# anyboby/Constrained-Model-Based-Policy-Optimization

Hardware: NVIDIA B200
Metric: model-rollout transitions/sec (higher is better)
Workload: dtype f16 (tcgen05 kind::f16, f32 accumulate)

## Files before the change

### constrained-model-based-policy-optimization_b200/csrc/common.cuh

```cuda
#pragma once
#include <cuda_runtime.h>
#include <stdint.h>
#include <stdio.h>
#include <string>
#include <vector>

#include "../../include/cmbpo_b200.h"

#define CMBPO_MAX_LAYERS 8
#define CMBPO_MAX_E 8
#define CMBPO_MAX_OBS 64
#define CMBPO_MAX_ACT 32

void cmbpo_set_error(const char* fmt, ...);

#define CUDA_TRY(expr)                                                                   \
    do {                                                                                 \
        cudaError_t _e = (expr);                                                         \
        if (_e != cudaSuccess) {                                                         \
            cmbpo_set_error("%s failed: %s (%s:%d)", #expr, cudaGetErrorString(_e), __FILE__, \
                            __LINE__);                                                   \
            return 1;                                                                    \
        }                                                                                \
    } while (0)
// ... 66 lines not shown
    ProfScope(cmbpo_ctx* c, int s) : ctx(c), slot(s), on(c->profile && s >= 0) {
        if (!on) return;
        ProfSlot& p = ctx->prof[slot];
        if (p.used == p.start.size()) {
            cudaEvent_t a, b;
            cudaEventCreate(&a); cudaEventCreate(&b);
            p.start.push_back(a); p.stop.push_back(b);
        }
        cudaEventRecord(p.start[p.used], ctx->stream);
    }
    ~ProfScope() {
        if (!on) return;
        ProfSlot& p = ctx->prof[slot];
        cudaEventRecord(p.stop[p.used], ctx->stream);
        p.used++;
    }
};

static inline int cdiv(int64_t a, int64_t b) { return (int)((a + b - 1) / b); }

int ens_forward_f32(cmbpo_ctx* ctx, const Net& net, const float* x, int64_t N, bool x_is_3d,
                    float* out_raw);
struct FusedStep;
int ens_forward_tc(cmbpo_ctx* ctx, Net& net, const float* x, int64_t N, float* out_raw,
                   int precision, const int64_t* n_dev = nullptr, const FusedStep* fz = nullptr);
bool ens_tc_fusable(const Net& net);
int ens_tc_fused_rp_shift(int obs_dim);
bool ens_tc_supported(const Net& net);
int ens_tc_prepare(cmbpo_ctx* ctx, Net& net);
int policy_pack_build(cmbpo_ctx* ctx);
void net_free(Net& n);
void train_free(cmbpo_ctx* ctx, int which);
int ens_forward(cmbpo_ctx* ctx, Net& net, const float* x, int64_t N, bool x_is_3d, float* out_raw,
                int precision, const int64_t* n_dev = nullptr);
```

### constrained-model-based-policy-optimization_b200/csrc/ens_tc.cu

```cuda
#include <cstring>
#include "tc_common.cuh"
#include "step_common.cuh"

using namespace tc;

namespace {

constexpr int NTHREADS = 640;
constexpr int TILE = 8192;
constexpr int STAGE = 4 * TILE;
constexpr int NSM = 5;
constexpr int W2SLOT = 16384;
constexpr int NS2 = 2;
constexpr int BIAS_SLOT = 4096;
constexpr int XA_BYTES = 16384;

struct Stage {
    int layer, n0, k0, rows, member;
    unsigned long long off;
};

struct TcParams {
    const uint8_t* wmain; unsigned long long main_bytes;
    const uint8_t* w2; unsigned long long w2_bytes;
    const float* bias; int bias_stride;
    int E, K0, KS0, Nout, NP, parts, cps;
    int fold;
    const float* x; long long N; int ldx;
    const long long* n_dev;
    const float *mu_in, *sig_in;
    float* out; long long out_member_stride;
    int ntiles;
    int member_act[CMBPO_MAX_E];
    FusedStep fz;
};

enum { W_FULL = 0, W_EMPTY = NSM, W2_FULL = 2 * NSM, W2_EMPTY = 2 * NSM + NS2, D_FULL = 2 * NSM + 2 * NS2,
       D_EMPTY = D_FULL + 2, H1_FULL = D_FULL + 4, H2_FULL = D_FULL + 5, H2_EMPTY = D_FULL + 7,
       OUT_FULL = D_FULL + 9, OUT_EMPTY = D_FULL + 10, X_FULL = D_FULL + 11, B_FULL = D_FULL + 12,
       B_EMPTY = D_FULL + 14, NBAR = D_FULL + 16 };
constexpr int HL_FULL = H2_FULL;
static_assert(H2_EMPTY == H2_FULL + 2, "HL_FULL spans the H2_FULL and H2_EMPTY pairs");
constexpr int SMEM_W2 = XA_BYTES + NSM * STAGE;
constexpr int SMEM_BIAS = SMEM_W2 + NS2 * W2SLOT;
constexpr int SMEM_IN_BYTES = 512;
constexpr int SMEM_BAR = SMEM_BIAS + 2 * BIAS_SLOT + SMEM_IN_BYTES;
constexpr int SMEM_TOTAL = SMEM_BAR + NBAR * 8 + 16;
constexpr int W2SLOT_F = 12288;
constexpr int FZ_STAGE = 12288, FZ_MISC = 5120;
constexpr int SMEM_BIAS_F = SMEM_W2 + NS2 * W2SLOT_F;
constexpr int SMEM_BAR_F = SMEM_BIAS_F + 2 * BIAS_SLOT + SMEM_IN_BYTES;
constexpr int SMEM_FZ = SMEM_BAR_F + NBAR * 8 + 16;
constexpr int SMEM_TOTAL_F = SMEM_FZ + FZ_STAGE + FZ_MISC;
static_assert(SMEM_FZ % 16 == 0 && SMEM_TOTAL_F + 1024 <= 232448, "fused shared-memory budget");

struct FzSmem {
    float *kl, *epv;
    int *member, *path;
    int* nonfin;
    float* spec;
    float *sig, *mu, *l2s;
    float* log_std;
    int* elite;
    unsigned char* state;
    int* flag;
};
__device__ __forceinline__ FzSmem fz_views(uint8_t* base) {
    FzSmem m;
    m.kl = reinterpret_cast<float*>(base);
    m.epv = nullptr;
// ... 96 lines not shown
            if (!c.deterministic)
                eps = f.state_eps ? f.state_eps[pth * O + dim] : philox_normal(f.seed, f.path_base + pth, t, RNG_STREAM_STATE, dim);
            RawTile raw(tbase, W, r0 + rr);
            const float ob = f.cur_obs[(base + rr) * O + dim];
            const float nx = env_dim_nx<true>(c, raw, dim, member, ob, eps);
            if (!f.rules.no_store) {
                f.rules.b.obs[row * O + dim] = ob;
                f.rules.b.nextobs[row * O + dim] = nx;
            }
            f.cur_obs[(base + rr) * O + dim] = nx;
        }
        if (!f.rules.no_store)
        for (int idx = etid; idx < RP * A; idx += 512) {
            const int rr = idx / A, i = idx - rr * A;
            if (sm.state[rr] != 1) continue;
            const long long pth = sm.path[rr], row = (long long)t * f.rules.B + pth;
            f.rules.b.act[row * A + i] = f.pi[(base + rr) * A + i];
            f.rules.b.mu[row * A + i] = f.mu[(base + rr) * A + i];
        }
        epi_bar();
    }
}


template <int FMT, int ACT>
__device__ __forceinline__ void drain32(uint32_t d_addr, const float* bias, uint32_t dst_addr,
                                        uint32_t d_empty, uint32_t dst_free, uint32_t dst_parity,
                                        bool rt_swish = false) {
    uint32_t r[32];
    tmem_ld32(d_addr, r);
    tmem_ld_wait();
    tc_fence_before();
    __syncwarp();
    if ((threadIdx.x & 31) == 0) mbar_arrive_a(d_empty);
    uint32_t q[16];
    float v[32];
    if (bias) {
#pragma unroll
        for (int i = 0; i < 32; i += 4) {
            const float4 b = *reinterpret_cast<const float4*>(bias + i);
            v[i] = __uint_as_float(r[i]) + b.x; v[i + 1] = __uint_as_float(r[i + 1]) + b.y;
            v[i + 2] = __uint_as_float(r[i + 2]) + b.z; v[i + 3] = __uint_as_float(r[i + 3]) + b.w;
        }
    } else {
#pragma unroll
        for (int i = 0; i < 32; ++i) v[i] = __uint_as_float(r[i]);
    }
#pragma unroll
    for (int i = 0; i < 32; ++i) {
        if (ACT == 0) {
            const float r = tanh_approx(v[i]);
            const float sw = fmaf(v[i], r, v[i]);
            v[i] = rt_swish ? sw : r;
        } else {
            v[i] = (ACT == CMBPO_ACT_SWISH) ? swish_half(v[i]) : tanh_approx(v[i]);
        }
    }
#pragma unroll
    for (int c = 0; c < 16; ++c) q[c] = Cvt<FMT>::pack(v[2 * c], v[2 * c + 1]);
    if (dst_free) { mbar_wait_a(dst_free, dst_parity); tc_fence_after(); }
    tmem_st16(dst_addr, q);
    tmem_st_wait();
    tc_fence_before();
}

template <int HD, int FMT, int ACT, int G, bool FUSE, int NMID = 0, int CL = 1, bool WO = false>
__global__ void __launch_bounds__(NTHREADS, 1) ens_mlp3_tc_kernel(const TcParams p) {
    static_assert(CL == 1 || (CL == 2 && G == 1 && !FUSE), "cluster pairs: ordinary ensembles only");
    static_assert(!FUSE || G == 1, "the fused step kernel exists for ordinary (ungrouped) ensembles");
    static_assert(NMID == 0 || (HD <= 256 && G == 1 && !FUSE), "deep variant: width <= 256, ungrouped");
    static_assert(!WO || (NMID > 0 && HD == 256 && CL == 1), "wide-output variant: deep nets at padded width 256");
    constexpr int W2S = FUSE ? W2SLOT_F : W2SLOT;
    constexpr int NC = HD / 64;
    constexpr int KP = HD / 64 / G;
    constexpr int CPM = NC / G;
    constexpr int TPS = KP < 4 ? KP : 4;
    constexpr int G0 = NC < 4 ? NC : 4;
    constexpr uint32_t COL_H1 = 0, COL_D = HD / 2, COL_H2 = COL_D + 128;
    constexpr uint32_t COL_HB = WO ? COL_H2 : COL_H2 + 64;
    constexpr int NHID = 1 + NMID;
    constexpr uint32_t COL_LAST = ((NMID + 1) & 1) ? COL_HB : COL_H1;
    extern __shared__ uint8_t smem_raw[];
    uint8_t* smem = reinterpret_cast<uint8_t*>((reinterpret_cast<uintptr_t>(smem_raw) + 1023) & ~uintptr_t(1023));
    uint8_t* sXA = smem;
    uint8_t* sW = smem + XA_BYTES;
    uint8_t* sW2 = smem + SMEM_W2;
    float* sBias = reinterpret_cast<float*>(smem + (FUSE ? SMEM_BIAS_F : SMEM_BIAS));
    float* sIn = sBias + 2 * BIAS_SLOT / 4;
    constexpr int BAR_OFF = FUSE ? SMEM_BAR_F : SMEM_BAR;
    uint64_t* bar = reinterpret_cast<uint64_t*>(smem + BAR_OFF);
// ... 226 lines not shown
                }
                ++m;
            }
        }
        }
        __syncwarp();
    }
    } else {
        asm volatile("setmaxnreg.inc.sync.aligned.u32 112;");
        const int wg = (warp - 4) >> 2;
        const uint32_t pair = (uint32_t)wg >> 1, half = (uint32_t)wg & 1;
        const int wq = hw_warp & 3;
        const int row = wq * 32 + lane;
        const uint32_t lane_base = (uint32_t)(wq * 32) << 16;
        const uint32_t bar_a = smem_u32(bar);
        uint32_t g = 0, m = 0, c1 = 0;
        int prev_e = 0; long long prev_grow = 0; uint32_t prev_m = 0; bool have_prev = false;
        int prev_tile = 0;
        const int etid = (int)threadIdx.x - 128;
        if (etid < 64) {
            sIn[etid] = (p.mu_in && etid < p.K0) ? p.mu_in[etid] : 0.f;
            sIn[64 + etid] = (p.mu_in && etid < p.K0) ? p.sig_in[etid] : 1.f;
        }
        epi_bar();
        FzSmem fsm;
        if (FUSE) {
            fsm = fz_views(smem + SMEM_FZ);
            const FusedStep& f = p.fz;
            for (int i = etid; i < f.c.D; i += 512) { fsm.sig[i] = f.c.sig_out[i]; fsm.mu[i] = f.c.mu_out[i]; fsm.l2s[i] = f.c.l2s_out[i]; }
            if (etid < f.A) fsm.log_std[etid] = f.log_std[etid];
            if (etid < f.n_elite && etid < 8) fsm.elite[etid] = f.c.elite[etid];
            epi_bar();
        }
        const int out_cw = (G > 1) ? p.NP : ((p.NP <= 64) ? 16 : 32);
        auto out_epilogue = [&]() {
            mbar_wait(bar + OUT_FULL, prev_m & 1);
            tc_fence_after();
            const int c_begin = wg * out_cw;
            uint32_t r[32];
            const bool mine = (G > 1) ? (wg < G && prev_e * G + wg < p.E) : (c_begin < p.NP);
            if (mine) {
                tmem_ld16(tmem + col_out + c_begin + lane_base, *reinterpret_cast<uint32_t(*)[16]>(&r[0]));
                if (out_cw == 32) tmem_ld16(tmem + col_out + c_begin + 16 + lane_base, *reinterpret_cast<uint32_t(*)[16]>(&r[16]));
                tmem_ld_wait();
            }
            tc_fence_before();
            __syncwarp();
            if (lane == 0) mbar_arrive(bar + OUT_EMPTY);
            if (FUSE) {
                const FusedStep& f = p.fz;
                if (mine) {
                    const float* b2 = p.bias + (long long)prev_e * p.bias_stride + (1 + NHID) * HD;
                    float* dst = f.raw_tiles + ((size_t)prev_tile * p.E + prev_e) * p.Nout * 128 + row;
#pragma unroll
                    for (int i = 0; i < 32; ++i) {
                        const int c = c_begin + i;
                        if (i < out_cw && c < p.Nout) __stcg(dst + (size_t)c * 128, __uint_as_float(r[i]) + __ldg(b2 + c));
                    }
                }
                __threadfence();
                epi_bar();
                if (etid == 0) {
                    const int old = atomicAdd(f.tile_cnt + prev_tile, 1);
                    const int last = (old == p.E - 1) ? 1 : 0;
                    if (last) f.tile_cnt[prev_tile] = 0;
                    *fsm.flag = last;
                }
                epi_bar();
                if (*fsm.flag) {
                    __threadfence();
                    fused_rows(f, fsm, prev_tile, n_rows, etid);
// ... 240 lines not shown
        for (int j = 0; j < NC; ++j)
            for (int kp = 0; kp < KPm; ++kp) {
                main_prog->push_back(Stage{lyr, (j % CPM) * 64, kp * 64, 64, j / CPM, off});
                off += TILE;
            }
    *main_bytes = off;
    off = 0;
    for (int j = 0; j < NC; ++j)
        for (int q = 0; q < parts; ++q) {
            w2_prog->push_back(Stage{nhid + 1, q * NPp, (j % CPM) * 64, NPp, j / CPM, off});
            off += (unsigned long long)NPp * 128;
        }
    *w2_bytes = off;
}

int chunks_per_w2_slot(int HD, int NP, int slot_bytes = W2SLOT) {
    int cps = slot_bytes / (NP * 128);
    int p2 = 1;
    while (p2 * 2 <= cps) p2 *= 2;
    const int NC = HD / 64;
    return p2 < NC ? p2 : NC;
}

template <int HD, int FMT, int ACT, int G = 1, bool FUSE = false, int NMID = 0, bool WO = false>
int launch_tc(cmbpo_ctx* ctx, const TcParams& p) {
    const int smem = (FUSE ? SMEM_TOTAL_F : SMEM_TOTAL) + 1024;
    static_assert(SMEM_TOTAL + 1024 <= 232448, "shared memory budget");
    auto kern = ens_mlp3_tc_kernel<HD, FMT, ACT, G, FUSE, NMID, 1, WO>;
    CUDA_TRY(cudaFuncSetAttribute(kern, cudaFuncAttributeMaxDynamicSharedMemorySize, smem));
    const long long units = (long long)p.ntiles * ((p.E + G - 1) / G);
    const int grid = units < ctx->sm_count ? (int)units : ctx->sm_count;
    kern<<<grid, NTHREADS, smem, ctx->stream>>>(p);
    ctx->launches++;
    CUDA_TRY(cudaGetLastError());
    return 0;
}

template <int HD, int FMT, int ACT>
int launch_tc_pairs(cmbpo_ctx* ctx, const TcParams& p) {
    const int smem = SMEM_TOTAL + 1024;
    auto kern = ens_mlp3_tc_kernel<HD, FMT, ACT, 1, false, 0, 2>;
    static int max_pairs = -1;
    cudaLaunchConfig_t cfg = {};
    cudaLaunchAttribute attr[1];
    attr[0].id = cudaLaunchAttributeClusterDimension;
    attr[0].val.clusterDim.x = 2; attr[0].val.clusterDim.y = 1; attr[0].val.clusterDim.z = 1;
    cfg.blockDim = dim3(NTHREADS); cfg.dynamicSmemBytes = smem; cfg.stream = ctx->stream;
    cfg.attrs = attr; cfg.numAttrs = 1;
    if (max_pairs < 0) {
        CUDA_TRY(cudaFuncSetAttribute(kern, cudaFuncAttributeMaxDynamicSharedMemorySize, smem));
        cfg.gridDim = dim3(2 * (ctx->sm_count / 2));
// ... 24 lines not shown

template <int HD, int FMT>
int launch_tc_act(cmbpo_ctx* ctx, const TcParams& p, int act) {
    if (act == 0) return launch_tc<HD, FMT, 0>(ctx, p);
    if (act == CMBPO_ACT_SWISH) return launch_tc<HD, FMT, CMBPO_ACT_SWISH>(ctx, p);
    return launch_tc<HD, FMT, CMBPO_ACT_TANH>(ctx, p);
}

template <int FMT, int ACT, int NMID>
int launch_tc_deep_out(cmbpo_ctx* ctx, const TcParams& p) {
    if (p.NP > 64) return launch_tc<256, FMT, ACT, 1, false, NMID, true>(ctx, p);
    return launch_tc<256, FMT, ACT, 1, false, NMID>(ctx, p);
}
template <int FMT>
int launch_tc_deep(cmbpo_ctx* ctx, const TcParams& p, int act, int nmid) {
    if (act == CMBPO_ACT_SWISH)
        return nmid == 1 ? launch_tc_deep_out<FMT, CMBPO_ACT_SWISH, 1>(ctx, p)
                         : launch_tc_deep_out<FMT, CMBPO_ACT_SWISH, 2>(ctx, p);
    return nmid == 1 ? launch_tc_deep_out<FMT, CMBPO_ACT_TANH, 1>(ctx, p)
                     : launch_tc_deep_out<FMT, CMBPO_ACT_TANH, 2>(ctx, p);
}

template <int FMT>
int launch_tc_grouped(cmbpo_ctx* ctx, const TcParams& p, int act) {
    if (act == 0) return launch_tc<512, FMT, 0, 4>(ctx, p);
    if (act == CMBPO_ACT_SWISH) return launch_tc<512, FMT, CMBPO_ACT_SWISH, 4>(ctx, p);
    return launch_tc<512, FMT, CMBPO_ACT_TANH, 4>(ctx, p);
}

template <int FMT>
int launch_tc_hd(cmbpo_ctx* ctx, const TcParams& p, int hd, int act) {
    if (hd == 128) return launch_tc_act<128, FMT>(ctx, p, act);
    if (hd == 256) return launch_tc_act<256, FMT>(ctx, p, act);
    if (p.ntiles >= 2) {
        if (act == CMBPO_ACT_SWISH) return launch_tc_pairs<512, FMT, CMBPO_ACT_SWISH>(ctx, p);
        return launch_tc_pairs<512, FMT, CMBPO_ACT_TANH>(ctx, p);
    }
    if (act == CMBPO_ACT_SWISH) return launch_tc<512, FMT, CMBPO_ACT_SWISH>(ctx, p);
    return launch_tc<512, FMT, CMBPO_ACT_TANH>(ctx, p);
}

}

bool ens_tc_supported(const Net& n) {
    if (!n.loaded || n.n_layers < 3 || n.n_layers > 5) return false;
    const int hd = n.dims[1], L = n.n_layers;
    for (int l = 1; l < L; ++l) if (n.dims[l] != hd) return false;
// ... 31 lines not shown
        const size_t total = (size_t)n_units * (main_bytes + w2_bytes);
        CUDA_TRY(cudaMalloc(&net.tc_pack[prec], total));
        net.tc_pack_bytes[prec] = (size_t)main_bytes;
        uint8_t* base = (uint8_t*)net.tc_pack[prec];
        uint8_t* base2 = base + (size_t)n_units * main_bytes;
        dim3 g1((unsigned)mp.size(), n_units), g2((unsigned)wp.size(), n_units);
        if (prec == CMBPO_PREC_FP16) {
            pack_weights_kernel<0><<<g1, 256, 0, ctx->stream>>>(pw, net.b[0], K0, HR, Nout, net.E, group, d_mp, (int)mp.size(), main_bytes, pc, base);
            pack_weights_kernel<0><<<g2, 256, 0, ctx->stream>>>(pw, net.b[0], K0, HR, Nout, net.E, group, d_wp, (int)wp.size(), w2_bytes, pc, base2);
        } else {
            pack_weights_kernel<1><<<g1, 256, 0, ctx->stream>>>(pw, net.b[0], K0, HR, Nout, net.E, group, d_mp, (int)mp.size(), main_bytes, pc, base);
            pack_weights_kernel<1><<<g2, 256, 0, ctx->stream>>>(pw, net.b[0], K0, HR, Nout, net.E, group, d_wp, (int)wp.size(), w2_bytes, pc, base2);
        }
    }
    CUDA_TRY(cudaMalloc(&net.tc_bias, (size_t)n_units * group * ((L - 1) * HD + os.NP) * sizeof(float)));
    pack_bias_kernel<<<n_units, 256, 0, ctx->stream>>>(pb, HD, HR, Nout, os.NP, net.E, group, pc, net.tc_bias);
    CUDA_TRY(cudaStreamSynchronize(ctx->stream));
    CUDA_TRY(cudaFree(d_mp));
    CUDA_TRY(cudaFree(d_wp));
    CUDA_TRY(cudaGetLastError());
    return 0;
}

bool ens_tc_fusable(const Net& n) {
    if (!ens_tc_supported(n) || n.n_layers != 3 || n.tc_group != 1 || n.E != 7 || !n.probabilistic) return false;
    if (n.acts[0] != CMBPO_ACT_SWISH || n.member_act[0] >= 0) return false;
    const OutShape os = out_shape(n.dims[3]);
    return os.NP * 128 <= W2SLOT_F && n.D <= 64;
}

int ens_tc_fused_rp_shift(int O) {
    int sh = 7;
    while (sh > 5 && (size_t)(1 << sh) * O * 8 > (size_t)FZ_STAGE) --sh;
    return ((size_t)(1 << sh) * O * 8 <= (size_t)FZ_STAGE) ? sh : -1;
}

int ens_forward_tc(cmbpo_ctx* ctx, Net& net, const float* x, int64_t N, float* out_raw, int precision,
                   const int64_t* n_dev, const FusedStep* fz) {
    CMBPO_CHECK(precision == CMBPO_PREC_BF16 || precision == CMBPO_PREC_FP16, "bad precision %d", precision);
    CMBPO_CHECK(net.tc_pack[precision], "tcgen05 weights not packed");
    if (N <= 0) return 0;
    CMBPO_CHECK((N + 127) / 128 * (int64_t)net.E < (int64_t)1 << 31, "too many rows for one launch");
    const int HD = net.tc_hd;
    const int nmid = net.n_layers - 3;
    const OutShape os = out_shape(net.dims[net.n_layers]);
    TcParams p;
    p.Nout = net.dims[net.n_layers];
    p.NP = os.NP; p.parts = os.parts;
    p.cps = chunks_per_w2_slot(HD * net.tc_group, os.NP, fz ? W2SLOT_F : W2SLOT);
    p.wmain = (const uint8_t*)net.tc_pack[precision];
    p.main_bytes = net.tc_pack_bytes[precision];
    p.w2 = p.wmain + (size_t)((net.E + net.tc_group - 1) / net.tc_group) * p.main_bytes;
    p.w2_bytes = (unsigned long long)(HD * net.tc_group / 64) * p.NP * 128;
    const int group = net.tc_group;
    p.bias = net.tc_bias; p.bias_stride = group * ((net.n_layers - 1) * HD + p.NP);
    p.E = net.E; p.K0 = net.dims[0]; p.fold = net.tc_fold; p.KS0 = (p.K0 + (p.fold ? 2 : 0) + 15) / 16;
    p.x = x; p.N = N; p.ldx = net.dims[0];
    p.n_dev = reinterpret_cast<const long long*>(n_dev);
    p.mu_in = net.has_in ? net.mu_in : nullptr; p.sig_in = net.sig_in;
    p.out = out_raw; p.out_member_stride = (long long)N * p.Nout;
    p.ntiles = (int)((N + 127) / 128);
    for (int i = 0; i < CMBPO_MAX_E; ++i) p.member_act[i] = net.member_act[i];
    if (fz) {
        CMBPO_CHECK(ens_tc_fusable(net) && fz->rp_shift >= 5, "this ensemble cannot run the fused rollout step");
        p.fz = *fz;
        return precision == CMBPO_PREC_FP16 ? launch_tc_fused<0>(ctx, p, HD) : launch_tc_fused<1>(ctx, p, HD);
    }
    memset(&p.fz, 0, sizeof(p.fz));
    const int act_sel = net.member_act[0] >= 0 ? 0 : net.acts[0];
    if (nmid > 0) {
        CMBPO_CHECK(HD == 256 && group == 1 && (nmid == 1 || nmid == 2) && net.member_act[0] < 0, "deep tcgen05 variant: bad shape");
        return precision == CMBPO_PREC_FP16 ? launch_tc_deep<0>(ctx, p, act_sel, nmid) : launch_tc_deep<1>(ctx, p, act_sel, nmid);
    }
    if (group == 4) return precision == CMBPO_PREC_FP16 ? launch_tc_grouped<0>(ctx, p, act_sel) : launch_tc_grouped<1>(ctx, p, act_sel);
    if (precision == CMBPO_PREC_FP16) return launch_tc_hd<0>(ctx, p, HD, act_sel);
    return launch_tc_hd<1>(ctx, p, HD, act_sel);
}
```

### constrained-model-based-policy-optimization_b200/csrc/rollout.cu

```cuda
#include <cstdlib>
#include <cstring>
#include "common.cuh"
#include "row_math.cuh"
#include "step_common.cuh"

namespace {

struct PolicyRowsArgs {
    int64_t N;
    int O, A;
    const float* obs;
    const float* mu_raw;
    const float* log_std;
    ValueHead v, vc;
    const float* eps;
    const int32_t* path_ids;
    int64_t path_base;
    uint64_t seed;
    int step;
    const uint8_t* alive;
    const int32_t* row_path;
    const int64_t* n_dev;
    float *pi, *logp, *mu, *vout, *vcout;
    float* xin;
// ... 235 lines not shown
            const int r = idx / O, dim = idx - r * O;
            const int member = s_member[r];
            if (member < 0) continue;
            const int64_t p = s_path[r];
            float eps = 1.0f;
            if (!a.c.deterministic)
                eps = a.state_eps ? a.state_eps[p * O + dim]
                                  : philox_normal(a.seed, a.path_base + p, t, RNG_STREAM_STATE, dim);
            RawStaged raw(s_raw, rows, W, r);
            const EnvDimOut d = env_dim<EC, FAST>(a.c, raw, dim, member, a.cur_obs[(base + r) * O + dim], eps);
            s_kl[idx] = d.kl; s_epv[idx] = d.epv; s_nx[idx] = d.nx;
            s_fin[idx] = isfinite(d.nx) ? 1 : 0;
        }
        __syncthreads();
        if (threadIdx.x < rows && s_member[threadIdx.x] >= 0) {
            const int r = threadIdx.x;
            const int64_t p = s_path[r];
            RawStaged raw(s_raw, rows, W, r);
            const EnvRowOut o = env_row_finish<FAST>(a.c, raw, s_member[r], s_kl + r * O, s_epv + r * O, s_nx + r * O,
                                               s_fin + r * O);
            RowCarry pf;
            pf.v = pf_v; pf.vc = pf_vc; pf.logp = pf_logp; pf.dkl = pf_dkl; pf.ret = pf_ret; pf.cost = pf_cost;
            s_state[r] = (unsigned char)step_row_commit(a.rules, p, o, pf, st0, st1, st2, st3);
        }
        __syncthreads();
        for (int idx = threadIdx.x; idx < NI; idx += STEP_THREADS) {
            const int r = idx / O, dim = idx - r * O;
            if (s_state[r] != 1) continue;
            const int64_t p = s_path[r], row = (int64_t)t * a.B + p;
            const float nx = s_nx[idx];
            if (!a.rules.no_store) {
                a.b.obs[row * O + dim] = a.cur_obs[(base + r) * O + dim];
                a.b.nextobs[row * O + dim] = nx;
            }
            a.cur_obs[(base + r) * O + dim] = nx;
        }
        if (!a.rules.no_store)
        for (int idx = threadIdx.x; idx < rows * A; idx += STEP_THREADS) {
            const int r = idx / A, i = idx - r * A;
            if (s_state[r] != 1) continue;
            const int64_t p = s_path[r], row = (int64_t)t * a.B + p;
            a.b.act[row * A + i] = a.pi[(base + r) * A + i];
            a.b.mu[row * A + i] = a.mu[(base + r) * A + i];
        }
        __syncthreads();
    }
// ... 70 lines not shown
    c.kl_closed_form = (precision != CMBPO_PREC_FP32) ? 1 : 0;
    c.sig_out = dyn.sig_out; c.mu_out = dyn.mu_out; c.l2s_out = dyn.l2s_out; c.elite = dyn.elite;
    return c;
}

ValueHead make_head(const Net& n, const float* raw) {
    ValueHead h;
    h.raw = raw; h.E = n.E; h.ld = 1;
    h.mu_out = n.has_out ? n.mu_out : nullptr; h.sig_out = n.sig_out;
    return h;
}

int check_dyn(const cmbpo_ctx* ctx, const cmbpo_env_cfg* cfg, int O) {
    const Net& dyn = ctx->nets[CMBPO_NET_DYN];
    CMBPO_CHECK(dyn.loaded && dyn.probabilistic, "dynamics ensemble not loaded (or not probabilistic)");
    CMBPO_CHECK(dyn.has_out, "dynamics ensemble needs an output scaler");
    CMBPO_CHECK(dyn.E <= CMBPO_MAX_E, "at most %d ensemble members", CMBPO_MAX_E);
    CMBPO_CHECK(O <= CMBPO_MAX_OBS, "obs dim %d > %d", O, CMBPO_MAX_OBS);
    CMBPO_CHECK(dyn.D == O + 1 + (cfg->predicts_cost ? 1 : 0), "model output width %d does not match obs dim %d", dyn.D, O);
    CMBPO_CHECK(dyn.n_elite > 0, "no elite indices");
    return 0;
}

int policy_forward(cmbpo_ctx* ctx, PolicyRowsArgs a, bool with_actor, int precision) {
    Net& actor = ctx->nets[CMBPO_NET_ACTOR];
    Net& v = ctx->nets[CMBPO_NET_V];
    Net& vc = ctx->nets[CMBPO_NET_VC];
    CMBPO_CHECK(v.loaded && vc.loaded, "value ensembles not loaded");
    if (precision != CMBPO_PREC_FP32 && ctx->polnet.loaded) {
        Net& pn = ctx->polnet;
        const int A = pn.dims[3];
        CMBPO_CHECK(ctx->log_std && A <= CMBPO_MAX_ACT, "actor not loaded");
        float* raw;
        if (cmbpo_ws_get(ctx, 3, (size_t)pn.E * a.N * A * sizeof(float), (void**)&raw)) return 1;
        if (ens_forward(ctx, pn, a.obs, a.N, false, raw, precision, a.n_dev)) return 1;
        a.mu_raw = with_actor ? raw : nullptr;
        a.log_std = ctx->log_std;
        a.v = make_head(v, raw + (size_t)a.N * A); a.v.ld = A;
        a.vc = make_head(vc, raw + (size_t)(1 + v.E) * a.N * A); a.vc.ld = A;
        policy_rows_kernel<true><<<cdiv(a.N, POLICY_ROWS), POLICY_THREADS, 0, ctx->stream>>>(a);
        ctx->launches++;
        CUDA_TRY(cudaGetLastError());
        return 0;
    }
    float *raw_v, *raw_vc, *raw_mu = nullptr;
    if (cmbpo_ws_get(ctx, 3, (size_t)(v.E + vc.E) * a.N * sizeof(float), (void**)&raw_v)) return 1;
    raw_vc = raw_v + (size_t)v.E * a.N;
    const int pv = (precision != CMBPO_PREC_FP32 && ens_tc_supported(v)) ? precision : CMBPO_PREC_FP32;
    const int pvc = (precision != CMBPO_PREC_FP32 && ens_tc_supported(vc)) ? precision : CMBPO_PREC_FP32;
    if (ens_forward(ctx, v, a.obs, a.N, false, raw_v, pv)) return 1;
    if (ens_forward(ctx, vc, a.obs, a.N, false, raw_vc, pvc)) return 1;
    if (with_actor) {
        CMBPO_CHECK(actor.loaded && ctx->log_std, "actor not loaded");
        CMBPO_CHECK(a.A <= CMBPO_MAX_ACT, "act dim too large");
        if (cmbpo_ws_get(ctx, 4, (size_t)a.N * a.A * sizeof(float), (void**)&raw_mu)) return 1;
// ... 150 lines not shown
            fz.vc = make_head(ctx->nets[CMBPO_NET_VC], pol_raw + (size_t)(1 + ctx->nets[CMBPO_NET_V].E) * B * A); fz.vc.ld = A;
            fz.log_std = ctx->log_std;
            fz.pi = pi; fz.mu = mu; fz.logp = logp; fz.vrow = v; fz.vcrow = vc;
            fz.act_eps = bufs->act_eps ? bufs->act_eps + (size_t)t * B * A : nullptr;
            fz.elite_pos = bufs->elite_pos ? bufs->elite_pos + (size_t)t * B : nullptr;
            fz.state_eps = bufs->state_eps ? bufs->state_eps + (size_t)t * B * O : nullptr;
            fz.row_path = compacting ? row_path[cur_gen] : nullptr;
            fz.raw_tiles = raw; fz.tile_cnt = tile_cnt; fz.rp_shift = rp_shift;
            {
                ProfScope prof(ctx, CMBPO_PROF_DYN);
                if (ens_forward_tc(ctx, dyn, nullptr, B, nullptr, cfg->precision, nd, &fz)) return 1;
            }
        } else {
        PolicyRowsArgs pa = {};
        pa.N = B; pa.O = O; pa.A = A; pa.obs = cur;
        pa.row_path = compacting ? row_path[cur_gen] : nullptr;
        pa.n_dev = compacting ? n_dev + cur_gen : nullptr;
        pa.eps = (bufs->act_eps && !last) ? bufs->act_eps + (size_t)t * B * A : nullptr;
        pa.path_base = cfg->path_id_base; pa.seed = cfg->seed; pa.step = t;
        pa.alive = alive; pa.pi = pi; pa.logp = logp; pa.mu = mu; pa.vout = v; pa.vcout = vc;
        pa.xin = xin; pa.pending = pending; pa.last_val = bufs->last_val; pa.last_cval = bufs->last_cval;
        {
            ProfScope prof(ctx, CMBPO_PROF_POLICY);
            if (policy_forward(ctx, pa, !last, cfg->precision)) return 1;
        }
        if (last) break;
        if (ens_forward(ctx, dyn, xin, B, false, raw, cfg->precision, pa.n_dev)) return 1;
        StepArgs sa = {};
        sa.row_path = pa.row_path; sa.n_dev = pa.n_dev;
        sa.B = B; sa.O = O; sa.A = A; sa.T = T; sa.t = t;
        sa.c = make_env_cfg(dyn, cfg->env, O, cfg->precision); sa.n_elite = dyn.n_elite;
        sa.rules.B = B; sa.rules.t = t; sa.rules.last_storable = T - 2;
        sa.rules.uncertainty = cfg->uncertainty_mode; sa.rules.dkl_lim = cfg->dkl_lim;
        sa.rules.alive = alive; sa.rules.pending = pending; sa.rules.b = *bufs;
        sa.rules.no_store = (cfg->flags & CMBPO_ROLLOUT_NO_STORE) ? 1 : 0;
        sa.path_base = cfg->path_id_base; sa.seed = cfg->seed;
        sa.raw = raw; sa.cur_obs = cur; sa.alive = alive;
        sa.pi = pi; sa.mu = mu; sa.logp = logp; sa.v = v; sa.vc = vc;
        sa.elite_pos = bufs->elite_pos ? bufs->elite_pos + (size_t)t * B : nullptr;
        sa.state_eps = bufs->state_eps ? bufs->state_eps + (size_t)t * B * O : nullptr;
        sa.b = *bufs;
        {
            const size_t smem = step_smem_bytes(O, dyn.E, 2 * dyn.D);
            const bool fast = sa.c.kl_closed_form && sa.c.E == 7;
            if (!fast) sa.c.kl_closed_form = 0;
            auto kern = fast ? rollout_step_kernel<7, true> : rollout_step_kernel<0, false>;
            if (smem > ctx->step_smem_max[fast]) {
// ... 188 lines not shown
```

### constrained-model-based-policy-optimization_b200/csrc/step_common.cuh

```cuda
#pragma once
#include "common.cuh"
#include "row_math.cuh"

struct ValueHead {
    const float* raw;
    int E, ld;
    const float *mu_out, *sig_out;
};

__device__ __forceinline__ float value_of(const ValueHead& h, int64_t N, int64_t p) {
    float s = 0.f;
    for (int e = 0; e < h.E; ++e) {
        float m = h.raw[((int64_t)e * N + p) * h.ld];
        if (h.mu_out) m = __fadd_rn(__fmul_rn(h.sig_out[0], m), h.mu_out[0]);
        s = (e == 0) ? m : __fadd_rn(s, m);
    }
    return __fdiv_rn(s, (float)h.E);
}

template <bool FAST>
__device__ __forceinline__ float policy_head_row(const float* mu_row, const float* log_std, const float* eps_row,
                                                 uint64_t seed, int64_t gid, int step, int A, float* pi_row,
                                                 float* mu_out_row, float* pi_out_row2 = nullptr) {
    NpSumStream acc(A);
    float z0 = 0.f, z1 = 0.f, z2 = 0.f, z3 = 0.f;
    for (int a = 0; a < A; ++a) {
        if (!eps_row && (a & 3) == 0) {
            uint32_t o[4];
            philox4x32_10((uint32_t)gid, (uint32_t)((uint64_t)gid >> 32), (uint32_t)step,
                          ((uint32_t)RNG_STREAM_ACT << 16) | (uint32_t)(a >> 2), (uint32_t)seed,
                          (uint32_t)(seed >> 32), o);
            box_muller(o[0], o[1], z0, z1);
            if (a + 2 < A) box_muller(o[2], o[3], z2, z3);
        }
        const int k = a & 3;
        const float eps = eps_row ? eps_row[a] : (k == 0 ? z0 : (k == 1 ? z1 : (k == 2 ? z2 : z3)));
        const float mu = mu_row[a];
        float pi;
        acc.add(a, actor_dim<FAST>(mu, log_std[a], eps, pi));
        if (pi_row) pi_row[a] = pi;
        if (mu_out_row) mu_out_row[a] = mu;
        if (pi_out_row2) pi_out_row2[a] = pi;
    }
    return acc.result();
}

struct StepRules {
    int64_t B; int t, last_storable;
    int uncertainty; double dkl_lim;
    int no_store;
    uint8_t* alive;
    uint8_t* pending;
    cmbpo_rollout_bufs b;
};

struct RowCarry { float v, vc, logp; double dkl, ret, cost; };

__device__ __forceinline__ int step_row_commit(const StepRules& a, int64_t p, const EnvRowOut& o, const RowCarry& pf,
                                               double& st0, double& st1, double& st2, double& st3) {
    const float v = pf.v, vc = pf.vc;
    const double next_dkl = pf.dkl + (double)o.dkl_path;
    const bool cut = a.uncertainty && next_dkl >= a.dkl_lim;
    st0 += 1.0; st1 += (double)o.dkl_path;
    if (cut) {
        a.alive[p] = 0;
        a.b.end_reason[p] = CMBPO_END_UNCERTAIN;
        a.b.last_val[p] = v; a.b.last_cval[p] = vc;
// ... 19 lines not shown
    }
    return 1;
}

struct FusedStep {
    StepRules rules;
    int O, A, n_elite;
    EnvRowCfg c;
    int64_t path_base; uint64_t seed;
    float* cur_obs;
    const float* pol_raw;
    ValueHead v, vc;
    const float* log_std;
    float *pi, *mu, *logp, *vrow, *vcrow;
    const float* act_eps;
    const int32_t* elite_pos;
    const float* state_eps;
    const int32_t* row_path;
    float* raw_tiles;
    int* tile_cnt;
    int rp_shift;
};

struct RawTile {
    const float* row0; int estride;
    __device__ RawTile(const float* tile_base, int W, int r) : row0(tile_base + r), estride(W * 128) {}
    __device__ float operator()(int e, int c) const { return __ldcg(row0 + e * estride + c * 128); }
    __device__ const float* ptr(int c) const { return row0 + c * 128; }
    __device__ static float load(const float* q) { return __ldcg(q); }
};
```

### constrained-model-based-policy-optimization_b200/csrc/tc_common.cuh

```cuda
#pragma once
#include <cuda_bf16.h>
#include <cuda_fp16.h>

#include "common.cuh"

namespace tc {

__device__ __forceinline__ uint32_t smem_u32(const void* p) {
    return (uint32_t)__cvta_generic_to_shared(p);
}

__device__ __forceinline__ bool elect_one() {
    uint32_t pred;
    asm volatile(
        "{\n\t.reg .pred p;\n\t"
        "elect.sync _|p, 0xffffffff;\n\t"
        "selp.u32 %0, 1, 0, p;\n\t}"
        : "=r"(pred));
    return pred != 0;
}

__device__ __forceinline__ void mbar_init(uint64_t* bar, uint32_t count) {
    asm volatile("mbarrier.init.shared::cta.b64 [%0], %1;" ::"r"(smem_u32(bar)), "r"(count));
}
// ... 111 lines not shown
}
__device__ __forceinline__ void tmem_ld32(uint32_t taddr, uint32_t (&r)[32]) {
    asm volatile(
        "tcgen05.ld.sync.aligned.32x32b.x32.b32 "
        "{%0, %1, %2, %3, %4, %5, %6, %7, %8, %9, %10, %11, %12, %13, %14, %15, "
        "%16, %17, %18, %19, %20, %21, %22, %23, %24, %25, %26, %27, %28, %29, %30, %31}, [%32];"
        : "=r"(r[0]), "=r"(r[1]), "=r"(r[2]), "=r"(r[3]), "=r"(r[4]), "=r"(r[5]), "=r"(r[6]),
          "=r"(r[7]), "=r"(r[8]), "=r"(r[9]), "=r"(r[10]), "=r"(r[11]), "=r"(r[12]), "=r"(r[13]),
          "=r"(r[14]), "=r"(r[15]), "=r"(r[16]), "=r"(r[17]), "=r"(r[18]), "=r"(r[19]), "=r"(r[20]),
          "=r"(r[21]), "=r"(r[22]), "=r"(r[23]), "=r"(r[24]), "=r"(r[25]), "=r"(r[26]), "=r"(r[27]),
          "=r"(r[28]), "=r"(r[29]), "=r"(r[30]), "=r"(r[31])
        : "r"(taddr)
        : "memory");
}
__device__ __forceinline__ void tmem_ld16(uint32_t taddr, uint32_t (&r)[16]) {
    asm volatile(
        "tcgen05.ld.sync.aligned.32x32b.x16.b32 "
        "{%0, %1, %2, %3, %4, %5, %6, %7, %8, %9, %10, %11, %12, %13, %14, %15}, [%16];"
        : "=r"(r[0]), "=r"(r[1]), "=r"(r[2]), "=r"(r[3]), "=r"(r[4]), "=r"(r[5]), "=r"(r[6]),
          "=r"(r[7]), "=r"(r[8]), "=r"(r[9]), "=r"(r[10]), "=r"(r[11]), "=r"(r[12]), "=r"(r[13]),
          "=r"(r[14]), "=r"(r[15])
        : "r"(taddr)
        : "memory");
}
__device__ __forceinline__ void tmem_ld_wait() {
    asm volatile("tcgen05.wait::ld.sync.aligned;" ::: "memory");
}

__device__ __forceinline__ uint64_t smem_desc_sw128(uint32_t smem_addr) {
    return (uint64_t)((smem_addr & 0x3FFFFu) >> 4) | (1ull << 16) | (64ull << 32) | (1ull << 46) |
           (2ull << 61);
}
__host__ __device__ constexpr uint32_t idesc_f16(int fmt, int n) {
    return (1u << 4) | ((uint32_t)fmt << 7) | ((uint32_t)fmt << 10) | ((uint32_t)(n >> 3) << 17) |
           ((uint32_t)(128 >> 4) << 24);
}

__host__ __device__ constexpr uint32_t panel_off(int r, int c) {
    return (uint32_t)((r >> 3) * 1024 + (r & 7) * 128 + ((c ^ (r & 7)) << 4));
}

template <int FMT> struct Cvt;
template <> struct Cvt<0> {
    __device__ static uint32_t pack(float a, float b) {
        uint32_t d;
        asm("cvt.rn.satfinite.f16x2.f32 %0, %1, %2;" : "=r"(d) : "f"(b), "f"(a));
// ... 77 lines not shown
```

Measured before the change: 157.2 million.

## Fuse policy/value heads into grouped tcgen05 policy MLP epilogue

Adds a HEAD variant of the grouped tcgen05 MLP kernel whose epilogue computes actor sampling, log-prob, value and cost-value means, and writes the dynamics input rows directly from TMEM accumulators. This removes the raw output buffer round-trip and the separate policy/value head kernel launches per rollout step. In exchange it adds extra TMEM loads and per-warp head work in the epilogue, and moves clearing of pending flags into the step kernel. It applies only to non-last steps and to specific ensemble shapes.

Result: no change. 157.4 million (median of 6 runs) (+0.1%).

```diff
diff --git a/constrained-model-based-policy-optimization_b200/csrc/common.cuh b/constrained-model-based-policy-optimization_b200/csrc/common.cuh
--- a/constrained-model-based-policy-optimization_b200/csrc/common.cuh
+++ b/constrained-model-based-policy-optimization_b200/csrc/common.cuh
@@ -112,8 +112,11 @@
 int ens_forward_f32(cmbpo_ctx* ctx, const Net& net, const float* x, int64_t N, bool x_is_3d,
                     float* out_raw);
 struct FusedStep;
+struct PolicyHead;
 int ens_forward_tc(cmbpo_ctx* ctx, Net& net, const float* x, int64_t N, float* out_raw,
-                   int precision, const int64_t* n_dev = nullptr, const FusedStep* fz = nullptr);
+                   int precision, const int64_t* n_dev = nullptr, const FusedStep* fz = nullptr,
+                   const PolicyHead* ph = nullptr);
+bool ens_tc_policy_head(const Net& polnet, int nv, int nvc);
 bool ens_tc_fusable(const Net& net);
 int ens_tc_fused_rp_shift(int obs_dim);
 bool ens_tc_supported(const Net& net);
diff --git a/constrained-model-based-policy-optimization_b200/csrc/ens_tc.cu b/constrained-model-based-policy-optimization_b200/csrc/ens_tc.cu
--- a/constrained-model-based-policy-optimization_b200/csrc/ens_tc.cu
+++ b/constrained-model-based-policy-optimization_b200/csrc/ens_tc.cu
@@ -33,6 +33,7 @@
     int ntiles;
     int member_act[CMBPO_MAX_E];
     FusedStep fz;
+    PolicyHead ph;
 };
 
 enum { W_FULL = 0, W_EMPTY = NSM, W2_FULL = 2 * NSM, W2_EMPTY = 2 * NSM + NS2, D_FULL = 2 * NSM + 2 * NS2,
@@ -46,6 +47,7 @@
 constexpr int SMEM_IN_BYTES = 512;
 constexpr int SMEM_BAR = SMEM_BIAS + 2 * BIAS_SLOT + SMEM_IN_BYTES;
 constexpr int SMEM_TOTAL = SMEM_BAR + NBAR * 8 + 16;
+constexpr int SMEM_TOTAL_H = SMEM_TOTAL + 64;
 constexpr int W2SLOT_F = 12288;
 constexpr int FZ_STAGE = 12288, FZ_MISC = 5120;
 constexpr int SMEM_BIAS_F = SMEM_W2 + NS2 * W2SLOT_F;
@@ -188,6 +190,53 @@
     }
 }
 
+__device__ __forceinline__ void head_epilogue(const PolicyHead& h, const uint32_t* acc, const uint32_t (&vacc)[4],
+                                              int gm, int nvh, int wg, int NP, const float* b2, const float* log_std,
+                                              long long grow, long long n_rows) {
+    const long long pth = (grow < n_rows) ? (h.row_path ? (long long)h.row_path[grow] : grow) : -1;
+    if (gm == 0) {
+        const int A = h.A, O = h.O;
+        if (pth >= 0 && h.alive[pth])
+            h.logp[grow] = policy_head_row<true>(
+                [&](int a) {
+                    float x = __uint_as_float(acc[0]);
+#pragma unroll
+                    for (int k = 1; k < 16; ++k) if (a == k) x = __uint_as_float(acc[k]);
+                    return __fadd_rn(x, b2[a]);
+                },
+                log_std, h.act_eps ? h.act_eps + pth * A : nullptr, h.seed, h.path_base + pth, h.t, A,
+                h.pi + grow * A, h.mu + grow * A, h.xin + grow * (O + A) + O);
+    } else if (gm == 3) {
+        const int O = h.O, W = O + h.A;
+        const bool live = pth >= 0 && h.alive[pth];
+        const int lane = (int)threadIdx.x & 31;
+        const long long wrow = grow - lane;
+        for (int i0 = 0; i0 < 32 * W; i0 += 32 * 8) {
+            float x[8];
+            int dst[8];
+#pragma unroll
+            for (int j = 0; j < 8; ++j) {
+                const int idx = i0 + 32 * j + lane, rr = idx / W, c = idx - rr * W;
+                const bool lv = __shfl_sync(0xffffffffu, live, rr & 31);
+                dst[j] = (idx < 32 * W && lv && c < O) ? rr * W + c : -1;
+                if (dst[j] >= 0) x[j] = h.obs[(wrow + rr) * O + c];
+            }
+#pragma unroll
+            for (int j = 0; j < 8; ++j)
+                if (dst[j] >= 0) h.xin[wrow * W + dst[j]] = x[j];
+        }
+    }
+    if (nvh > 0 && pth >= 0) {
+        const bool is_v = gm == 1;
+        const float val = value_mean(is_v ? h.v : h.vc, [&](int e) {
+            const uint32_t x = e == 0 ? vacc[0] : (e == 1 ? vacc[1] : (e == 2 ? vacc[2] : vacc[3]));
+            return __fadd_rn(__uint_as_float(x), b2[(wg + e) * NP]);
+        });
+        if (h.pending[pth] & (is_v ? 1 : 2)) (is_v ? h.last_val : h.last_cval)[pth] = val;
+        if (h.alive[pth]) (is_v ? h.vrow : h.vcrow)[grow] = val;
+    }
+}
+
 
 template <int FMT, int ACT>
 __device__ __forceinline__ void drain32(uint32_t d_addr, const float* bias, uint32_t dst_addr,
@@ -230,8 +279,9 @@
     tc_fence_before();
 }
 
-template <int HD, int FMT, int ACT, int G, bool FUSE, int NMID = 0, int CL = 1, bool WO = false>
+template <int HD, int FMT, int ACT, int G, bool FUSE, int NMID = 0, int CL = 1, bool WO = false, bool HEAD = false>
 __global__ void __launch_bounds__(NTHREADS, 1) ens_mlp3_tc_kernel(const TcParams p) {
+    static_assert(!HEAD || (HD == 512 && G == 4 && ACT == 0 && !FUSE && NMID == 0 && CL == 1), "policy head: grouped merged policy pass");
     static_assert(CL == 1 || (CL == 2 && G == 1 && !FUSE), "cluster pairs: ordinary ensembles only");
     static_assert(!FUSE || G == 1, "the fused step kernel exists for ordinary (ungrouped) ensembles");
     static_assert(NMID == 0 || (HD <= 256 && G == 1 && !FUSE), "deep variant: width <= 256, ungrouped");
@@ -504,6 +554,10 @@
             sIn[etid] = (p.mu_in && etid < p.K0) ? p.mu_in[etid] : 0.f;
             sIn[64 + etid] = (p.mu_in && etid < p.K0) ? p.sig_in[etid] : 1.f;
         }
+        float* sLogStd = reinterpret_cast<float*>(smem + SMEM_TOTAL);
+        if constexpr (HEAD) {
+            if (etid < p.ph.A) sLogStd[etid] = p.ph.log_std[etid];
+        }
         epi_bar();
         FzSmem fsm;
         if (FUSE) {
@@ -521,14 +575,30 @@
             const int c_begin = wg * out_cw;
             uint32_t r[32];
             const bool mine = (G > 1) ? (wg < G && prev_e * G + wg < p.E) : (c_begin < p.NP);
+            int gm = 0, nvh = 0;
+            uint32_t vacc[4];
+            if constexpr (HEAD) {
+                gm = prev_e * G + wg;
+                nvh = gm == 1 ? p.ph.v.E : (gm == 1 + p.ph.v.E ? p.ph.vc.E : 0);
+            }
             if (mine) {
                 tmem_ld16(tmem + col_out + c_begin + lane_base, *reinterpret_cast<uint32_t(*)[16]>(&r[0]));
                 if (out_cw == 32) tmem_ld16(tmem + col_out + c_begin + 16 + lane_base, *reinterpret_cast<uint32_t(*)[16]>(&r[16]));
+                if constexpr (HEAD) {
+#pragma unroll
+                    for (int k = 1; k < 4; ++k)
+                        if (k < nvh) tmem_ld1(tmem + col_out + (wg + k) * p.NP + lane_base, vacc[k]);
+                }
                 tmem_ld_wait();
+                if constexpr (HEAD) vacc[0] = r[0];
             }
             tc_fence_before();
             __syncwarp();
             if (lane == 0) mbar_arrive(bar + OUT_EMPTY);
+            if constexpr (HEAD) {
+                if (mine || gm == 3) head_epilogue(p.ph, r, vacc, gm, nvh, wg, p.NP, p.bias + (long long)prev_e * p.bias_stride + (1 + NHID) * HD,
+                                        sLogStd, prev_grow, n_rows);
+            } else
             if (FUSE) {
                 const FusedStep& f = p.fz;
                 if (mine) {
@@ -815,11 +885,11 @@
     return p2 < NC ? p2 : NC;
 }
 
-template <int HD, int FMT, int ACT, int G = 1, bool FUSE = false, int NMID = 0, bool WO = false>
+template <int HD, int FMT, int ACT, int G = 1, bool FUSE = false, int NMID = 0, bool WO = false, bool HEAD = false>
 int launch_tc(cmbpo_ctx* ctx, const TcParams& p) {
-    const int smem = (FUSE ? SMEM_TOTAL_F : SMEM_TOTAL) + 1024;
-    static_assert(SMEM_TOTAL + 1024 <= 232448, "shared memory budget");
-    auto kern = ens_mlp3_tc_kernel<HD, FMT, ACT, G, FUSE, NMID, 1, WO>;
+    const int smem = (FUSE ? SMEM_TOTAL_F : (HEAD ? SMEM_TOTAL_H : SMEM_TOTAL)) + 1024;
+    static_assert(SMEM_TOTAL_H + 1024 <= 232448, "shared memory budget");
+    auto kern = ens_mlp3_tc_kernel<HD, FMT, ACT, G, FUSE, NMID, 1, WO, HEAD>;
     CUDA_TRY(cudaFuncSetAttribute(kern, cudaFuncAttributeMaxDynamicSharedMemorySize, smem));
     const long long units = (long long)p.ntiles * ((p.E + G - 1) / G);
     const int grid = units < ctx->sm_count ? (int)units : ctx->sm_count;
@@ -890,7 +960,8 @@
 }
 
 template <int FMT>
-int launch_tc_grouped(cmbpo_ctx* ctx, const TcParams& p, int act) {
+int launch_tc_grouped(cmbpo_ctx* ctx, const TcParams& p, int act, bool head) {
+    if (head) return launch_tc<512, FMT, 0, 4, false, 0, false, true>(ctx, p);
     if (act == 0) return launch_tc<512, FMT, 0, 4>(ctx, p);
     if (act == CMBPO_ACT_SWISH) return launch_tc<512, FMT, CMBPO_ACT_SWISH, 4>(ctx, p);
     return launch_tc<512, FMT, CMBPO_ACT_TANH, 4>(ctx, p);
@@ -968,6 +1039,11 @@
     return 0;
 }
 
+bool ens_tc_policy_head(const Net& n, int nv, int nvc) {
+    return n.loaded && n.tc_group == 4 && n.n_layers == 3 && n.member_act[0] >= 0 && n.E == 1 + nv + nvc && nv >= 1 &&
+           nvc >= 1 && 1 + nv <= 4 && (1 + nv) / 4 == (nv + nvc) / 4;
+}
+
 bool ens_tc_fusable(const Net& n) {
     if (!ens_tc_supported(n) || n.n_layers != 3 || n.tc_group != 1 || n.E != 7 || !n.probabilistic) return false;
     if (n.acts[0] != CMBPO_ACT_SWISH || n.member_act[0] >= 0) return false;
@@ -982,7 +1058,7 @@
 }
 
 int ens_forward_tc(cmbpo_ctx* ctx, Net& net, const float* x, int64_t N, float* out_raw, int precision,
-                   const int64_t* n_dev, const FusedStep* fz) {
+                   const int64_t* n_dev, const FusedStep* fz, const PolicyHead* ph) {
     CMBPO_CHECK(precision == CMBPO_PREC_BF16 || precision == CMBPO_PREC_FP16, "bad precision %d", precision);
     CMBPO_CHECK(net.tc_pack[precision], "tcgen05 weights not packed");
     if (N <= 0) return 0;
@@ -1007,18 +1083,25 @@
     p.out = out_raw; p.out_member_stride = (long long)N * p.Nout;
     p.ntiles = (int)((N + 127) / 128);
     for (int i = 0; i < CMBPO_MAX_E; ++i) p.member_act[i] = net.member_act[i];
+    memset(&p.ph, 0, sizeof(p.ph));
     if (fz) {
         CMBPO_CHECK(ens_tc_fusable(net) && fz->rp_shift >= 5, "this ensemble cannot run the fused rollout step");
         p.fz = *fz;
         return precision == CMBPO_PREC_FP16 ? launch_tc_fused<0>(ctx, p, HD) : launch_tc_fused<1>(ctx, p, HD);
     }
     memset(&p.fz, 0, sizeof(p.fz));
+    if (ph) {
+        CMBPO_CHECK(ens_tc_policy_head(net, ph->v.E, ph->vc.E) && ph->A == p.Nout, "this policy pack cannot run the policy head");
+        p.ph = *ph;
+    }
     const int act_sel = net.member_act[0] >= 0 ? 0 : net.acts[0];
     if (nmid > 0) {
         CMBPO_CHECK(HD == 256 && group == 1 && (nmid == 1 || nmid == 2) && net.member_act[0] < 0, "deep tcgen05 variant: bad shape");
         return precision == CMBPO_PREC_FP16 ? launch_tc_deep<0>(ctx, p, act_sel, nmid) : launch_tc_deep<1>(ctx, p, act_sel, nmid);
     }
-    if (group == 4) return precision == CMBPO_PREC_FP16 ? launch_tc_grouped<0>(ctx, p, act_sel) : launch_tc_grouped<1>(ctx, p, act_sel);
+    if (group == 4)
+        return precision == CMBPO_PREC_FP16 ? launch_tc_grouped<0>(ctx, p, act_sel, ph != nullptr)
+                                            : launch_tc_grouped<1>(ctx, p, act_sel, ph != nullptr);
     if (precision == CMBPO_PREC_FP16) return launch_tc_hd<0>(ctx, p, HD, act_sel);
     return launch_tc_hd<1>(ctx, p, HD, act_sel);
 }
diff --git a/constrained-model-based-policy-optimization_b200/csrc/rollout.cu b/constrained-model-based-policy-optimization_b200/csrc/rollout.cu
--- a/constrained-model-based-policy-optimization_b200/csrc/rollout.cu
+++ b/constrained-model-based-policy-optimization_b200/csrc/rollout.cu
@@ -281,6 +281,8 @@
             RowCarry pf;
             pf.v = pf_v; pf.vc = pf_vc; pf.logp = pf_logp; pf.dkl = pf_dkl; pf.ret = pf_ret; pf.cost = pf_cost;
             s_state[r] = (unsigned char)step_row_commit(a.rules, p, o, pf, st0, st1, st2, st3);
+        } else if (threadIdx.x < rows && s_path[threadIdx.x] >= 0 && a.rules.pending[s_path[threadIdx.x]]) {
+            a.rules.pending[s_path[threadIdx.x]] = 0;
         }
         __syncthreads();
         for (int idx = threadIdx.x; idx < NI; idx += STEP_THREADS) {
@@ -397,7 +399,7 @@
     return 0;
 }
 
-int policy_forward(cmbpo_ctx* ctx, PolicyRowsArgs a, bool with_actor, int precision) {
+int policy_forward(cmbpo_ctx* ctx, PolicyRowsArgs a, bool with_actor, int precision, bool head_in_pass = false) {
     Net& actor = ctx->nets[CMBPO_NET_ACTOR];
     Net& v = ctx->nets[CMBPO_NET_V];
     Net& vc = ctx->nets[CMBPO_NET_VC];
@@ -406,6 +408,15 @@
         Net& pn = ctx->polnet;
         const int A = pn.dims[3];
         CMBPO_CHECK(ctx->log_std && A <= CMBPO_MAX_ACT, "actor not loaded");
+        if (head_in_pass && ens_tc_policy_head(pn, ctx->pol_nv, ctx->pol_nvc)) {
+            PolicyHead h = {};
+            h.O = a.O; h.A = A; h.t = a.step; h.path_base = a.path_base; h.seed = a.seed;
+            h.v = make_head(v, nullptr); h.vc = make_head(vc, nullptr);
+            h.obs = a.obs; h.log_std = ctx->log_std; h.act_eps = a.eps; h.row_path = a.row_path;
+            h.alive = a.alive; h.pending = a.pending; h.last_val = a.last_val; h.last_cval = a.last_cval;
+            h.pi = a.pi; h.mu = a.mu; h.logp = a.logp; h.vrow = a.vout; h.vcrow = a.vcout; h.xin = a.xin;
+            return ens_forward_tc(ctx, pn, a.obs, a.N, nullptr, precision, a.n_dev, nullptr, &h);
+        }
         float* raw;
         if (cmbpo_ws_get(ctx, 3, (size_t)pn.E * a.N * A * sizeof(float), (void**)&raw)) return 1;
         if (ens_forward(ctx, pn, a.obs, a.N, false, raw, precision, a.n_dev)) return 1;
@@ -602,7 +613,7 @@
         pa.xin = xin; pa.pending = pending; pa.last_val = bufs->last_val; pa.last_cval = bufs->last_cval;
         {
             ProfScope prof(ctx, CMBPO_PROF_POLICY);
-            if (policy_forward(ctx, pa, !last, cfg->precision)) return 1;
+            if (policy_forward(ctx, pa, !last, cfg->precision, !last)) return 1;
         }
         if (last) break;
         if (ens_forward(ctx, dyn, xin, B, false, raw, cfg->precision, pa.n_dev)) return 1;
diff --git a/constrained-model-based-policy-optimization_b200/csrc/step_common.cuh b/constrained-model-based-policy-optimization_b200/csrc/step_common.cuh
--- a/constrained-model-based-policy-optimization_b200/csrc/step_common.cuh
+++ b/constrained-model-based-policy-optimization_b200/csrc/step_common.cuh
@@ -8,18 +8,23 @@
     const float *mu_out, *sig_out;
 };
 
-__device__ __forceinline__ float value_of(const ValueHead& h, int64_t N, int64_t p) {
+template <class Raw>
+__device__ __forceinline__ float value_mean(const ValueHead& h, const Raw& raw) {
     float s = 0.f;
     for (int e = 0; e < h.E; ++e) {
-        float m = h.raw[((int64_t)e * N + p) * h.ld];
+        float m = raw(e);
         if (h.mu_out) m = __fadd_rn(__fmul_rn(h.sig_out[0], m), h.mu_out[0]);
         s = (e == 0) ? m : __fadd_rn(s, m);
     }
     return __fdiv_rn(s, (float)h.E);
 }
 
-template <bool FAST>
-__device__ __forceinline__ float policy_head_row(const float* mu_row, const float* log_std, const float* eps_row,
+__device__ __forceinline__ float value_of(const ValueHead& h, int64_t N, int64_t p) {
+    return value_mean(h, [&](int e) { return h.raw[((int64_t)e * N + p) * h.ld]; });
+}
+
+template <bool FAST, class MuOf>
+__device__ __forceinline__ float policy_head_row(const MuOf& mu_of, const float* log_std, const float* eps_row,
                                                  uint64_t seed, int64_t gid, int step, int A, float* pi_row,
                                                  float* mu_out_row, float* pi_out_row2 = nullptr) {
     NpSumStream acc(A);
@@ -35,7 +40,7 @@
         }
         const int k = a & 3;
         const float eps = eps_row ? eps_row[a] : (k == 0 ? z0 : (k == 1 ? z1 : (k == 2 ? z2 : z3)));
-        const float mu = mu_row[a];
+        const float mu = mu_of(a);
         float pi;
         acc.add(a, actor_dim<FAST>(mu, log_std[a], eps, pi));
         if (pi_row) pi_row[a] = pi;
@@ -43,6 +48,13 @@
         if (pi_out_row2) pi_out_row2[a] = pi;
     }
     return acc.result();
+}
+template <bool FAST>
+__device__ __forceinline__ float policy_head_row(const float* mu_row, const float* log_std, const float* eps_row,
+                                                 uint64_t seed, int64_t gid, int step, int A, float* pi_row,
+                                                 float* mu_out_row, float* pi_out_row2 = nullptr) {
+    return policy_head_row<FAST>([=](int a) { return mu_row[a]; }, log_std, eps_row, seed, gid, step, A, pi_row,
+                                 mu_out_row, pi_out_row2);
 }
 
 struct StepRules {
@@ -108,6 +120,20 @@
     int rp_shift;
 };
 
+struct PolicyHead {
+    int O, A, t;
+    int64_t path_base; uint64_t seed;
+    ValueHead v, vc;
+    const float* obs;
+    const float* log_std;
+    const float* act_eps;
+    const int32_t* row_path;
+    const uint8_t *alive, *pending;
+    float *last_val, *last_cval;
+    float *pi, *mu, *logp, *vrow, *vcrow;
+    float* xin;
+};
+
 struct RawTile {
     const float* row0; int estride;
     __device__ RawTile(const float* tile_base, int W, int r) : row0(tile_base + r), estride(W * 128) {}
diff --git a/constrained-model-based-policy-optimization_b200/csrc/tc_common.cuh b/constrained-model-based-policy-optimization_b200/csrc/tc_common.cuh
--- a/constrained-model-based-policy-optimization_b200/csrc/tc_common.cuh
+++ b/constrained-model-based-policy-optimization_b200/csrc/tc_common.cuh
@@ -157,6 +157,9 @@
           "=r"(r[14]), "=r"(r[15])
         : "r"(taddr)
         : "memory");
+}
+__device__ __forceinline__ void tmem_ld1(uint32_t taddr, uint32_t& r) {
+    asm volatile("tcgen05.ld.sync.aligned.32x32b.x1.b32 {%0}, [%1];" : "=r"(r) : "r"(taddr) : "memory");
 }
 __device__ __forceinline__ void tmem_ld_wait() {
     asm volatile("tcgen05.wait::ld.sync.aligned;" ::: "memory");
```
